# cvlab-kaist/PF3plat

Hardware: AMD Instinct MI355X
Metric: rendered views/sec, 300k Gaussians @ 256x256 (fwd raster); bwd ms and HBM GB/s vs roofline alongside (higher is better)
Workload: dtype f32; 1 GPU; configs[1]: 300000 Gaussians (SH degree 4, 25 coeffs), 1 view 256x256, fwd-only raster, one scene per GPU (seed 2+rank), inputs resident in HBM; launch=eager, parallelism=views sharded 1 scene/GPU x1, camera_setup=excluded (gsr_setup_views runs once before the loop; ~4 us per batch of views), num_pairs_8x8=1252130, max_tile_list=1663

## Files before the change

pf3plat_amd/csrc/gsr_tiles_fwd.h:

```cpp
#pragma once
#include "gsr_common.h"
#include "gsr_binning.h"

namespace gsr {

template <bool kFlip, class KeyPtr>
__device__ __forceinline__ void bitonic_substep(KeyPtr a, int n, int half, int lg, int tid) {
  constexpr int U = 4;
  const int w = 1 << lg;
  for (int tb = tid; tb < half; tb += kSortThreads * U) {
    int ii[U], jj[U];
    unsigned long long x[U], y[U];
    bool act[U];
#pragma unroll
    for (int u = 0; u < U; ++u) {
      const int t = tb + u * kSortThreads;
      const int blk = t >> lg, off = t & (w - 1);
      ii[u] = (blk << (lg + 1)) + off;
      jj[u] = kFlip ? (blk << (lg + 1)) + 2 * w - 1 - off : ii[u] + w;
      act[u] = (t < half) && (jj[u] < n);
      x[u] = act[u] ? a[ii[u]] : 0ull;
      y[u] = act[u] ? a[jj[u]] : 0ull;
    }
#pragma unroll
    for (int u = 0; u < U; ++u)
      if (act[u] && x[u] > y[u]) { a[ii[u]] = y[u]; a[jj[u]] = x[u]; }
  }
}

template <class KeyPtr>
__device__ __forceinline__ void bitonic_block(KeyPtr a, int n, int lgnp, int tid) {
  const int half = 1 << (lgnp - 1);
  for (int lk = 1; lk <= lgnp; ++lk) {
    bitonic_substep<true>(a, n, half, lk - 1, tid);
    __syncthreads();
    for (int lj = lk - 2; lj >= 0; --lj) {
      bitonic_substep<false>(a, n, half, lj, tid);
      __syncthreads();
    }
  }
}

constexpr int kSpanMax = 48;

__device__ __forceinline__ bool block_any(const bool pred, uint32_t* slot) {
  const bool w = __any((int)pred) != 0;
  if ((threadIdx.x & 63) == 0) slot[threadIdx.x >> 6] = w ? 1u : 0u;
  __syncthreads();
  return (slot[0] | slot[1] | slot[2] | slot[3]) != 0u;
}

__device__ __forceinline__ uint32_t block_exclusive_scan(uint32_t v, uint32_t* wave_tot , int tid, uint32_t& total) {
  const int lane = tid & 63, w = tid >> 6;
  const uint32_t s = wave_inclusive_scan_u32(v);
  if (lane == 63) wave_tot[w] = s;
  __syncthreads();
  uint32_t basew = 0;
  total = 0;
#pragma unroll
  for (int k = 0; k < kSortThreads / 64; ++k) {
    const uint32_t x = wave_tot[k];
    basew += (k < w) ? x : 0u;
    total += x;
  }
  return basew + s - v;
}

template <int kLds>
struct SortLds {
  static constexpr int kBuckets = kLds == 2048 ? 2048 : 1024, kBucketBits = kLds == 2048 ? 11 : 10;
  static constexpr int kWords = kLds + kBuckets / 2;
};

template <bool kGather, int kLds>
__device__ __forceinline__ uint2 sort_tile(const Params& p, const uint32_t bid, const int tg, unsigned long long* smem, uint32_t* red,
                                           uint32_t* sInfo) {
  constexpr int kBk = SortLds<kLds>::kBuckets, kBkBits = SortLds<kLds>::kBucketBits, kBpt = kBk / kSortThreads;
  static_assert(kLds == 4096 || kLds == 2048, "bucket geometry");
  unsigned long long* sk = smem;
  uint32_t* hist = reinterpret_cast<uint32_t*>(smem + kLds);
  uint32_t* cur = hist;
  const int tid = threadIdx.x;
  const bool dbg = GSR_ABL(p.d.flags, GSR_FLAG_DEBUG_TIMING);
  unsigned long long* stamp = dbg_stamps(p, 8192 + bid);
  unsigned long long* stamp2 = dbg_stamps(p, 8192 + p.sort_blocks + bid);
  GSR_STAMP(0);
  int n;
  uint32_t obase = 0;
  unsigned long long* keys;
  uint32_t* out;
  if (kGather) {
    const int T = p.g.T, R = p.rows;
    const int v = tg / T, t = tg - v * T;
    if (bid < 1024u) {
      for (int q = 0; q < (int)((bid >> kDephaseShift) % kDephaseGroups); ++q) __builtin_amdgcn_s_sleep(64);
    }
    const uint2* col = p.pair_mat + (size_t)v * R * (T + 8) + t;
    const size_t cstride = (size_t)T + 8;
    const uint32_t* bb = p.blk_base + (size_t)v * R;
    const bool one_stride = R <= kSortThreads;
    uint2 e0 = make_uint2(0u, 0u);
    uint32_t bb0 = 0, cnt_sum = 0, missing = 0;
    if (one_stride) {
      if (tid < R) { e0 = col[(size_t)tid * cstride]; bb0 = bb[tid]; }
      cnt_sum = e0.y;
      missing = (e0.y != 0u && bb0 == 0xffffffffu) ? 1u : 0u;
    } else {
      for (int r = tid; r < R; r += kSortThreads) {
        const uint32_t c = col[(size_t)r * cstride].y;
        cnt_sum += c;
        missing |= (c != 0u && bb[r] == 0xffffffffu) ? 1u : 0u;
      }
    }
    GSR_STAMP2(0);
    uint32_t total;
    const uint32_t start0 = block_exclusive_scan(cnt_sum, red, tid, total);
    __shared__ uint32_t sAnyMissing[kSortThreads / 64];
    const bool any_missing = block_any(missing, sAnyMissing);
    n = (int)total;
    const bool plain = !any_missing && (uint32_t)n <= p.stride && n <= kLds;
    if (!plain && tid == 64 && (uint32_t)n > p.status->max_list) atomicMax(&p.status->max_list, (uint32_t)n);
    if (plain) {
      if (tid == 0) p.ranges[tg] = make_uint2((uint32_t)tg * p.stride, (uint32_t)tg * p.stride + (uint32_t)n);
    } else if (tid == 0) {
      uint32_t rbase = (uint32_t)tg * p.stride, ok = any_missing ? 0u : 1u, scratch = 0;
      if (ok && (uint32_t)n > p.stride) {
        const uint32_t at = atomicAdd(p.tail_counter, (uint32_t)n);
        if (at <= p.tail_cap && (uint32_t)n <= p.tail_cap - at) rbase = p.tail_off + at;
        else ok = 0;
      }
      if (ok && n > kLds) {
        const uint32_t np = ((uint32_t)n + kPage - 1) / kPage;
        const uint32_t first = take_pages(p.page_counter_tiles, p.call_tag, np), half = p.key_pages / 2;
        if (first <= p.key_pages - half && np <= p.key_pages - half - first) scratch = p.pool_off + (half + first) * (uint32_t)kPage;
        else ok = 0;
      }
      if (!ok) p.status->overflow = 1u;
      p.ranges[tg] = ok ? make_uint2(rbase, rbase + (uint32_t)n) : make_uint2(0u, 0u);
      sInfo[0] = rbase; sInfo[1] = ok; sInfo[2] = scratch;
    }
    if (bid == 0) {
      unsigned long long part = 0;
      for (int k = tid; k < p.d.num_views * R; k += kSortThreads) part += p.blk_total[k];
      for (int o = 32; o > 0; o >>= 1) part += __shfl_down(part, o, 64);
      __shared__ unsigned long long sPart[kSortThreads / 64];
      if ((tid & 63) == 0) sPart[tid >> 6] = part;
      __syncthreads();
      if (tid == 0) p.status->num_pairs = sPart[0] + sPart[1] + sPart[2] + sPart[3];
    }
    uint32_t rbase = (uint32_t)tg * p.stride, scratch = 0;
    if (!plain) {
      __syncthreads();
      if (!sInfo[1]) return make_uint2(0u, 0u);
      rbase = sInfo[0]; scratch = sInfo[2];
    }
    obase = rbase;
    if (n == 0) return make_uint2(obase, obase);
    GSR_STAMP2(1);
    out = p.point_list + rbase;
    keys = p.keys + scratch;
    unsigned long long* dst = n > kLds ? keys : sk;
    auto copy_run = [&](const unsigned long long* src, uint32_t cnt, uint32_t start) {
      for (uint32_t j = 0; j < cnt; j += 6) {
        const ull2 a = *reinterpret_cast<const ull2*>(src + j);
        ull2 b = {0ull, 0ull}, c = {0ull, 0ull};
        if (j + 2 < cnt) b = *reinterpret_cast<const ull2*>(src + j + 2);
        if (j + 4 < cnt) c = *reinterpret_cast<const ull2*>(src + j + 4);
        unsigned long long* d = dst + start + j;
        d[0] = a.x;
        if (j + 1 < cnt) d[1] = a.y;
        if (j + 2 < cnt) d[2] = b.x;
        if (j + 3 < cnt) d[3] = b.y;
        if (j + 4 < cnt) d[4] = c.x;
        if (j + 5 < cnt) d[5] = c.y;
      }
    };
    if (one_stride) {
      if (e0.y) copy_run(p.keys + bb0 + e0.x, e0.y, start0);
      __syncthreads();
      GSR_STAMP2(2);
    } else {
      uint32_t carry = 0;
      for (int r0 = 0; r0 < R; r0 += kSortThreads) {
        const int r = r0 + tid;
        const uint2 e = r < R ? col[(size_t)r * cstride] : make_uint2(0u, 0u);
        uint32_t tot;
        const uint32_t start = carry + block_exclusive_scan(e.y, red, tid, tot);
        carry += tot;
        if (e.y) copy_run(p.keys + bb[r] + e.x, e.y, start);
        __syncthreads();
      }
    }
    if (n == 1) {
      if (tid == 0) out[0] = (uint32_t)dst[0];
      return make_uint2(obase, obase + 1u);
    }
  } else {
    const uint2 rg = p.ranges[bid];
    n = (int)(rg.y - rg.x);
    obase = rg.x;
    if (n == 0) return rg;
    keys = p.keys + rg.x;
    out = p.point_list + rg.x;
    if (n == 1) {
      if (tid == 0) out[0] = (uint32_t)keys[0];
      return rg;
    }
  }
  int lgnp = 1;
  while ((1 << lgnp) < n) ++lgnp;
  if (n > kLds) {
    __syncthreads();
    bitonic_block(keys, n, lgnp, tid);
    for (int k = tid; k < n; k += kSortThreads) out[k] = (uint32_t)keys[k];
    return make_uint2(obase, obase + (uint32_t)n);
  }
  constexpr int Q = kLds / kSortThreads;
  unsigned long long kreg[Q];
  uint32_t lo = 0xffffffffu, hi = 0u;
#pragma unroll
  for (int q = 0; q < Q; ++q) {
    const int k = tid + q * kSortThreads;
    kreg[q] = (k < n) ? (kGather ? sk[k] : keys[k]) : ~0ull;
    if (k < n) {
      const uint32_t d = (uint32_t)(kreg[q] >> 32);
      lo = d < lo ? d : lo;
      hi = d > hi ? d : hi;
    }
  }
  GSR_STAMP(1);
  for (int k = tid; k < kBk; k += kSortThreads) hist[k] = 0;
  hi = wave_max_u32(hi);
  lo = ~wave_max_u32(~lo);
  if ((tid & 63) == 0) { red[tid >> 6] = lo; red[4 + (tid >> 6)] = hi; }
  __syncthreads();
  lo = min(min(red[0], red[1]), min(red[2], red[3]));
  hi = max(max(red[4], red[5]), max(red[6], red[7]));
  const uint32_t range = hi - lo;
  const int shift = range < (uint32_t)kBk ? 0 : (32 - __clz((int)range)) - kBkBits;
#pragma unroll
  for (int q = 0; q < Q; ++q)
    if (tid + q * kSortThreads < n) atomicAdd(&hist[((uint32_t)(kreg[q] >> 32) - lo) >> shift], 1u);
  __syncthreads();
  GSR_STAMP(2);
  uint32_t c[kBpt], span = 0, cmax = 0;
#pragma unroll
  for (int q = 0; q < kBpt; ++q) { c[q] = hist[kBpt * tid + q]; span += c[q]; cmax = max(cmax, c[q]); }
  uint32_t total;
  uint32_t start = block_exclusive_scan(span, red, tid, total);
#pragma unroll
  for (int q = 0; q < kBpt; ++q) { cur[kBpt * tid + q] = start; start += c[q]; }
  __shared__ uint32_t sAnyBig[kSortThreads / 64];
  const bool big = block_any(cmax > (uint32_t)kSpanMax, sAnyBig);
  GSR_STAMP(3);
#pragma unroll
  for (int q = 0; q < Q; ++q)
    if (tid + q * kSortThreads < n) {
      const uint32_t slot = atomicAdd(&cur[((uint32_t)(kreg[q] >> 32) - lo) >> shift], 1u);
      sk[slot] = kreg[q];
    }
  __syncthreads();
  GSR_STAMP(4);
  if (!big) {
    for (int k = tid; k < n; k += kSortThreads) {
      const unsigned long long key = sk[k];
      const uint32_t b = ((uint32_t)(key >> 32) - lo) >> shift;
      const int bs = b ? (int)cur[b - 1] : 0, be = (int)cur[b];
      int rank = bs;
      for (int j = bs; j < be; j += 4) {
        const unsigned long long k0 = sk[j], k1 = sk[min(j + 1, be - 1)], k2 = sk[min(j + 2, be - 1)], k3 = sk[min(j + 3, be - 1)];
        rank += (k0 < key ? 1 : 0) + ((j + 1 < be && k1 < key) ? 1 : 0) + ((j + 2 < be && k2 < key) ? 1 : 0) +
                ((j + 3 < be && k3 < key) ? 1 : 0);
      }
      out[rank] = (uint32_t)key;
    }
    GSR_STAMP(5);
    GSR_STAMP(6);
    return make_uint2(obase, obase + (uint32_t)n);
  }
  bitonic_block(sk, n, lgnp, tid);
  __syncthreads();
  GSR_STAMP(5);
  for (int k = tid; k < n; k += kSortThreads) out[k] = (uint32_t)sk[k];
  GSR_STAMP(6);
  return make_uint2(obase, obase + (uint32_t)n);
}


constexpr float kLog2e = 1.4426950408889634f;
constexpr float kLn2 = 0.6931471805599453f;

__device__ __forceinline__ void to_exp2_domain(float4& q0, float4& q1) {
  q0.z = (-0.5f * kLog2e) * q0.z;
  q0.w = (-kLog2e) * q0.w;
  q1.x = (-0.5f * kLog2e) * q1.x;
}
__device__ __forceinline__ float splat_p2(float a2, float b2, float c2, float dx, float dy) {
  const float t = __builtin_fmaf(b2, dy, a2 * dx);
  return __builtin_fmaf(c2 * dy, dy, t * dx);
}

typedef float f2 __attribute__((ext_vector_type(2)));
constexpr int kFwdWaves = 4;
#ifndef GSR_KFS
#define GSR_KFS 8
#endif
constexpr int kFS = GSR_KFS;
constexpr int kFB = kFS * kFwdWaves;
constexpr int kFwdThreads = 64 * kFwdWaves;

__device__ __forceinline__ void stage_batch(const GeomRec* geom, const float4* rgbc, uint32_t n, uint32_t base, int lane,
                                            uint32_t id, bool want_extra, float4& g, float2& g2, float4& c) {
  g = make_float4(0, 0, 0, 0); g2 = make_float2(0, 0); c = make_float4(0, 0, 0, 0);
  if (base + lane < n) {
    const GeomRec* r = geom + id;
    const float4 q0 = r->q0, q1 = r->q1;
    const float4 col = rgbc[id];
    const float ex = want_extra ? q1.z : 0.f;
    g = q0; g2 = make_float2(q1.x, q1.y); c = make_float4(col.x, col.y, col.z, ex);
  }
}

struct BlendLds {
  float4 sXY[4][kFB / 2], sAB[4][kFB / 2], sCO[4][kFB / 2], sRG[4][kFB / 2], sBE[4][kFB / 2];
  float sP[2][kFwdWaves][64];
};
struct BlendFin {
  float sPart[kFwdWaves][5][64];
  uint32_t sLast[kFwdWaves][64];
};

struct BlendAcc {
  float Tb;
  float Tmin;
  f2 CR, CG, CB, CE;
  uint32_t last, consumed;
};

template <bool kExtra, bool kTight = false>
__device__ __forceinline__ bool blend_range(const GeomRec* geom, const float4* rgbc, const uint32_t* plist, const uint32_t n,
                                            const uint32_t b0, const uint32_t nbat, BlendLds& lds, BlendAcc& s, const float pxf,
                                            const float pyf) {
  auto& sXY = lds.sXY; auto& sAB = lds.sAB; auto& sCO = lds.sCO; auto& sRG = lds.sRG; auto& sBE = lds.sBE;
  auto& sP = lds.sP;
  const int wave = __builtin_amdgcn_readfirstlane((int)(threadIdx.x >> 6));
  const int lane = threadIdx.x & 63;
  float Tb = s.Tb, Tmin = s.Tmin;
  f2 al[kFS / 2];
  uint32_t last = s.last, consumed = s.consumed;
  const int e0 = wave * kFS;

  const f2 px2 = {pxf, pxf}, py2 = {pyf, pyf};
  f2 om[kFS / 2];
  auto eval = [&](uint32_t b) {
    const int gb = b & 3;
    f2 P2 = {1.f, 1.f};
#pragma unroll
    for (int u = 0; u < kFS; u += 2) {
      const float4 xy = sXY[gb][(e0 + u) >> 1], ab = sAB[gb][(e0 + u) >> 1], co = sCO[gb][(e0 + u) >> 1];
      const f2 dx = f2{xy.x, xy.y} - px2, dy = f2{xy.z, xy.w} - py2;
      const f2 a2 = {ab.x, ab.y}, b2 = {ab.z, ab.w}, c2 = {co.x, co.y}, o = {co.z, co.w};
      const f2 t = __builtin_elementwise_fma(b2, dy, a2 * dx);
      const f2 p2 = __builtin_elementwise_fma(c2 * dy, dy, t * dx);
      const f2 ao = o * f2{__builtin_amdgcn_exp2f(p2.x), __builtin_amdgcn_exp2f(p2.y)};
      const float alpha0 = fminf(0.99f, ao.x), alpha1 = fminf(0.99f, ao.y);
      const bool keep0 = !(p2.x > 0.f) && !(alpha0 < 1.0f / 255.0f), keep1 = !(p2.y > 0.f) && !(alpha1 < 1.0f / 255.0f);
      al[u >> 1] = f2{keep0 ? alpha0 : 0.f, keep1 ? alpha1 : 0.f};
      om[u >> 1] = f2{1.f, 1.f} - al[u >> 1];
      P2 *= om[u >> 1];
    }
    sP[b & 1][wave][lane] = P2.x * P2.y;
  };
  f2 CR = s.CR, CG = s.CG, CB = s.CB, CE = s.CE;
  auto accum = [&](uint32_t b, float Tf) {
    const int cb = b & 3;
    const bool alive_in = !(Tf < 0.0001f);
    float T = alive_in ? Tf : 0.f;
    float Tn[kFS];
    f2 w[kFS / 2];
    float Tp = T;
#pragma unroll
    for (int u = 0; u < kFS; u += 2) {
      Tn[u] = Tp * om[u >> 1].x;
      Tn[u + 1] = Tn[u] * om[u >> 1].y;
      Tp = Tn[u + 1];
    }
    const bool alive_out = !(Tp < 0.0001f);
    if (__any(alive_in && !alive_out)) {
      float Tq = T;
#pragma unroll
      for (int u = 0; u < kFS; u += 2) {
        const bool alive0 = !(Tn[u] < 0.0001f), alive1 = !(Tn[u + 1] < 0.0001f);
        w[u >> 1] = al[u >> 1] * f2{alive0 ? Tq : 0.f, alive1 ? Tn[u] : 0.f};
        Tq = Tn[u + 1];
        Tmin = alive0 ? Tn[u] : Tmin;
        Tmin = alive1 ? Tn[u + 1] : Tmin;
        last += (uint32_t)alive0 + (uint32_t)alive1;
      }
    } else {
      float Tq = T;
#pragma unroll
      for (int u = 0; u < kFS; u += 2) {
        w[u >> 1] = al[u >> 1] * f2{Tq, Tn[u]};
        Tq = Tn[u + 1];
      }
      Tmin = alive_out ? Tp : Tmin;
      last += alive_out ? (uint32_t)kFS : 0u;
    }
#pragma unroll
    for (int u = 0; u < kFS; u += 2) {
      const float4 rg = sRG[cb][(e0 + u) >> 1], be = sBE[cb][(e0 + u) >> 1];
      CR = __builtin_elementwise_fma(f2{rg.x, rg.y}, w[u >> 1], CR);
      CG = __builtin_elementwise_fma(f2{rg.z, rg.w}, w[u >> 1], CG);
      CB = __builtin_elementwise_fma(f2{be.x, be.y}, w[u >> 1], CB);
      if (kExtra) CE = __builtin_elementwise_fma(f2{be.z, be.w}, w[u >> 1], CE);
    }
    asm volatile("" : "+v"(CR), "+v"(CG), "+v"(CB), "+v"(Tmin), "+v"(last));
    if (kExtra) asm volatile("" : "+v"(CE));
  };
  auto put_records = [&](int sb, float4 q, float2 q2, const float4& c) {
    q.z = (-0.5f * kLog2e) * q.z; q.w = (-kLog2e) * q.w; q2.x = (-0.5f * kLog2e) * q2.x;
    int ln = lane;
    if (kTight) asm volatile("" : "+v"(ln));
    const int o = (ln >> 1) * 4 + (ln & 1);
    float* xy = reinterpret_cast<float*>(sXY[sb]); float* ab = reinterpret_cast<float*>(sAB[sb]);
    float* co = reinterpret_cast<float*>(sCO[sb]); float* rg2 = reinterpret_cast<float*>(sRG[sb]);
    float* be = reinterpret_cast<float*>(sBE[sb]);
    xy[o] = q.x; xy[o + 2] = q.y; ab[o] = q.z; ab[o + 2] = q.w; co[o] = q2.x; co[o + 2] = q2.y;
    rg2[o] = c.x; rg2[o + 2] = c.y; be[o] = c.z; be[o + 2] = c.w;
  };

  bool done = false;
  if (nbat > b0) {
    float4 sg = make_float4(0, 0, 0, 0), sc = sg;
    float2 sg2 = make_float2(0, 0);
    uint32_t id_next = 0;
    int lp = lane;
    if (kTight) asm volatile("" : "+v"(lp));
    const auto list_id = [&](uint32_t b) { return (b * kFB + lp < n) ? plist[b * kFB + lp] : 0u; };
    if (lp < kFB) {
      const uint32_t w = (uint32_t)(wave - (int)b0) & 3u, bw = b0 + w;
      if (w < 2) {
        const uint32_t id0 = list_id(bw), id4 = list_id(bw + 4);
        id_next = list_id(bw + 8);
        if (bw < nbat) {
          stage_batch(geom, rgbc, n, bw * kFB, lane, id0, kExtra, sg, sg2, sc);
          put_records((int)(bw & 3), sg, sg2, sc);
        }
        stage_batch(geom, rgbc, n, (bw + 4) * kFB, lane, id4, kExtra, sg, sg2, sc);
      } else {
        const uint32_t id2 = list_id(bw);
        id_next = list_id(bw + 4);
        stage_batch(geom, rgbc, n, bw * kFB, lane, id2, kExtra, sg, sg2, sc);
      }
    }
    __syncthreads();
    eval(b0);
    __syncthreads();
    for (uint32_t i = b0; i < nbat; ++i) {
      const float P0 = sP[i & 1][0][lane], P1 = sP[i & 1][1][lane], P2 = sP[i & 1][2][lane], P3 = sP[i & 1][3][lane];
      const uint32_t bs = i + 2;
      const bool duty = (wave == (int)(bs & 3)) && (lane < kFB);
      const float t1 = Tb * P0, t2 = t1 * P1, t3 = t2 * P2, t4 = t3 * P3;
      const bool last_batch = __all(t4 < 0.0001f);
      accum(i, wave == 0 ? Tb : wave == 1 ? t1 : wave == 2 ? t2 : t3);
      if (i + 1 < nbat && !last_batch) eval(i + 1);
      if (duty) {
        if (bs < nbat) put_records((int)(bs & 3), sg, sg2, sc);
        if (bs + 4 < nbat) stage_batch(geom, rgbc, n, (bs + 4) * kFB, lane, id_next, kExtra, sg, sg2, sc);
        id_next = list_id(bs + 8);
      }
      Tb = t4;
      consumed = (i + 1) * kFB;
      __syncthreads();
      if (__all(Tb < 0.0001f)) { done = true; break; }
    }
  }
  s.Tb = Tb; s.Tmin = Tmin; s.CR = CR; s.CG = CG; s.CB = CB; s.CE = CE; s.last = last; s.consumed = consumed;
  return done;
}

template <bool kExtra, bool kAlpha = false>
__device__ __forceinline__ bool blend_poisoned(const Params& p, const int v, const int pxi, const int pyi, const bool inside,
                                               const bool known = false) {
  __shared__ uint32_t sAnyOverflow[kFwdThreads / 64];
  if (!known && !block_any(p.status->overflow != 0u, sAnyOverflow)) return false;
  const Grid& g = p.g;
  if (threadIdx.x < 64 && inside) {
    const size_t HW = (size_t)g.H * g.W, pix = (size_t)pyi * g.W + pxi;
    const float qnan = __uint_as_float(0x7fc00000u);
    float* oc = p.out_color + (size_t)v * 3 * HW;
    oc[pix] = qnan; oc[HW + pix] = qnan; oc[2 * HW + pix] = qnan;
    if (kExtra) p.out_extra[(size_t)v * HW + pix] = qnan;
    if (kAlpha) p.out_alpha[(size_t)v * HW + pix] = qnan;
    p.final_T[(size_t)v * HW + pix] = 1.f;
    p.n_contrib[(size_t)v * HW + pix] = 0u;
  }
  return true;
}

template <bool kExtra, bool kAlpha = false>
__device__ __forceinline__ void blend_finish(const Params& p, const int v, const int t, const uint32_t n, BlendFin& lds, const BlendAcc& s,
                                             const int pxi, const int pyi, const bool inside, const float bg0, const float bg1,
                                             const float bg2) {
  auto& sPart = lds.sPart; auto& sLast = lds.sLast;
  const Grid& g = p.g;
  const int wave = threadIdx.x >> 6, lane = threadIdx.x & 63;
  float C0 = s.CR.x + s.CR.y, C1 = s.CG.x + s.CG.y, C2 = s.CB.x + s.CB.y, E = s.CE.x + s.CE.y;
  sPart[wave][0][lane] = C0; sPart[wave][1][lane] = C1; sPart[wave][2][lane] = C2;
  if (kExtra) sPart[wave][3][lane] = E;
  sPart[wave][4][lane] = s.Tmin;
  sLast[wave][lane] = s.last;
  __syncthreads();
  if (wave == 0) {
    if (lane == 0) p.tile_total[(size_t)v * g.T + t] = min(s.consumed, n);
    if (inside) {
      float T = s.Tmin;
      uint32_t last = s.last;
#pragma unroll
      for (int h = 1; h < kFwdWaves; ++h) {
        C0 += sPart[h][0][lane]; C1 += sPart[h][1][lane]; C2 += sPart[h][2][lane];
        if (kExtra) E += sPart[h][3][lane];
        T = fminf(T, sPart[h][4][lane]);
        last += sLast[h][lane];
      }
      const size_t HW = (size_t)g.H * g.W, pix = (size_t)pyi * g.W + pxi;
      p.final_T[(size_t)v * HW + pix] = T;
      if (kAlpha) p.out_alpha[(size_t)v * HW + pix] = 1.f - T;
      p.n_contrib[(size_t)v * HW + pix] = min(last, n);
      float* oc = p.out_color + (size_t)v * 3 * HW;
      oc[pix] = C0 + T * bg0;
      oc[HW + pix] = C1 + T * bg1;
      oc[2 * HW + pix] = C2 + T * bg2;
      if (kExtra) p.out_extra[(size_t)v * HW + pix] = E;
    }
  }
}

template <bool kExtra, bool kAlpha = false>
__device__ __forceinline__ void blend_tile(const Params& p, const int v, const int t, const uint2 rg, BlendLds& lds) {
  const Grid& g = p.g;
  const int lane = threadIdx.x & 63;
  const int tx = t % g.sgx, ty = t / g.sgx;
  const int pxi = tx * 8 + (lane & 7), pyi = ty * 8 + (lane >> 3);
  const bool inside = pxi < g.W && pyi < g.H;
  const uint32_t n = rg.y - rg.x;
  typedef const __attribute__((address_space(4))) float* cfptr;
  cfptr camc = reinterpret_cast<cfptr>(reinterpret_cast<uintptr_t>(p.views + __builtin_amdgcn_readfirstlane(v)));
  const float bg0 = camc[37], bg1 = camc[38], bg2 = camc[39];
  if (blend_poisoned<kExtra, kAlpha>(p, v, pxi, pyi, inside)) return;
  const bool dbg = GSR_ABL(p.d.flags, GSR_FLAG_DEBUG_TIMING);
  unsigned long long tm0 = 0, rt0 = 0;
  if (dbg) { tm0 = __builtin_readcyclecounter(); rt0 = __builtin_amdgcn_s_memrealtime(); }
  BlendAcc acc;
  acc.Tb = inside ? 1.f : 0.f; acc.Tmin = 1.f;
  acc.CR = f2{0.f, 0.f}; acc.CG = acc.CR; acc.CB = acc.CR; acc.CE = acc.CR;
  acc.last = 0; acc.consumed = 0;
  (void)blend_range<kExtra>(p.geom + (size_t)v * p.d.num_gaussians, p.rgbc + (size_t)v * p.d.num_gaussians, p.point_list + rg.x, n, 0u,
                            (n + kFB - 1) / kFB, lds, acc, (float)pxi, (float)pyi);
  if (dbg && threadIdx.x == 0) {
    unsigned long long* o = dbg_stamps(p, 24576 + (size_t)v * g.T + t);
    const unsigned hw = (__builtin_amdgcn_s_getreg(4 | (0 << 6) | (15 << 11)) & 0xffffu) |
                        ((__builtin_amdgcn_s_getreg(20 | (0 << 6) | (15 << 11)) & 0xfu) << 16);
    o[0] = tm0; o[1] = ((unsigned long long)hw << 32); o[2] = __builtin_readcyclecounter();
    o[3] = (rt0 << 32) | (__builtin_amdgcn_s_memrealtime() & 0xffffffffull);
  }
  blend_finish<kExtra, kAlpha>(p, v, t, n, *reinterpret_cast<BlendFin*>(&lds + 1), acc, pxi, pyi, inside, bg0, bg1, bg2);
}

#ifndef GSR_TF_WAVES
#define GSR_TF_WAVES 6
#endif
#ifndef GSR_WINDOWED_SHORT
#define GSR_WINDOWED_SHORT 600
#endif
template <bool kGather, int kLds, bool kExtra, bool kAlpha = false>
__global__ __launch_bounds__(kFwdThreads, (kLds == 2048 && kGather && !kExtra) ? GSR_TF_WAVES : 4) void k_tile_fwd(const Params p) {
  static_assert(kSortThreads == kFwdThreads, "one workgroup shape for the two phases");
  constexpr int kSortWords = SortLds<kLds>::kWords, kBlendWords = (int)((sizeof(BlendLds) + sizeof(BlendFin) + 7) / 8);
  __shared__ __attribute__((aligned(16))) unsigned long long smem[kSortWords > kBlendWords ? kSortWords : kBlendWords];
  __shared__ uint32_t red[8];
  __shared__ uint32_t sInfo[4];
  const uint32_t bid = blockIdx.x;
  const int tg = kGather ? fwd_tile_of(p, fwd_tile_word(p, bid)) : (int)bid;
  __builtin_amdgcn_s_setprio(2);
  const uint2 rg = sort_tile<kGather, kLds>(p, bid, tg, smem, red, sInfo);
  __builtin_amdgcn_s_setprio(0);
  if (bid == 0 && threadIdx.x == 0) *p.page_counter = (unsigned long long)p.call_tag << 32;
  __syncthreads();
  const int v = tg / p.g.T;
  blend_tile<kExtra, kAlpha>(p, v, tg - v * p.g.T, rg, *reinterpret_cast<BlendLds*>(smem));
  if (kGather && threadIdx.x == 64 && rg.y - rg.x > p.status->max_list) atomicMax(&p.status->max_list, rg.y - rg.x);
}

#ifndef GSR_PREFIX
#define GSR_PREFIX 512
#endif
#ifndef GSR_DEPHASE_SLEEP
#define GSR_DEPHASE_SLEEP 16
#endif
#ifndef GSR_LONG_RUN
#define GSR_LONG_RUN 24
#endif
constexpr int kPrefix = GSR_PREFIX;
static_assert(kPrefix % kFB == 0 && kPrefix >= 2 * kFB, "the prefix is whole batches");

__device__ __forceinline__ uint2 sort_tile_general_2048(const Params& p, const uint32_t bid, const int tg, unsigned long long* smem, uint32_t* red, uint32_t* sInfo) {
  return sort_tile<true, 2048>(p, bid, tg, smem, red, sInfo);
}
__device__ __forceinline__ void bitonic_whole_list(unsigned long long* sk, uint32_t* out, const int n) {
  int lgnp = 1;
  while ((1 << lgnp) < n) ++lgnp;
  bitonic_block(sk, n, lgnp, (int)threadIdx.x);
  for (int k = threadIdx.x; k < n; k += kSortThreads) out[k] = (uint32_t)sk[k];
}

#ifndef GSR_PF_COMPACT_MIN_TILES
#define GSR_PF_COMPACT_MIN_TILES (5 * kCUs)
#endif
template <bool kExtra, bool kCompact, bool kAlpha = false>
__global__ __launch_bounds__(kFwdThreads, kCompact ? 6 : 4) void k_tile_fwd_prefix(const Params p) {
  constexpr int kLds = 2048;
  constexpr int kBk = kCompact ? 1024 : SortLds<kLds>::kBuckets, kBkBits = kCompact ? 10 : SortLds<kLds>::kBucketBits, kBpt = kBk / kSortThreads;
  constexpr int Q = kLds / kSortThreads;
  constexpr int kCounterWords = kCompact ? kBk / 4 : kBk / 2;
  constexpr int kBlendWordsP = (int)((sizeof(BlendLds) + 7) / 8);
  constexpr int kFastWords = kLds + kCounterWords + (kCompact ? kBlendWordsP : 0);
  __shared__ __attribute__((aligned(16))) unsigned long long smem[kFastWords > SortLds<kLds>::kWords ? kFastWords : SortLds<kLds>::kWords];
  __shared__ __attribute__((aligned(16))) unsigned long long blds_own[kCompact ? 2 : kBlendWordsP];
  BlendLds& blds = *reinterpret_cast<BlendLds*>(kCompact ? smem + kLds + kCounterWords : blds_own);
  __shared__ uint32_t red[8];
  __shared__ uint32_t sInfo[4];
  __shared__ uint32_t sCount, sLongRuns, sLongKeys;
  const uint32_t bid = blockIdx.x;
  const int tid = threadIdx.x, lane = tid & 63, wave = tid >> 6;
  const uint32_t tile_word = kCompact ? (uint32_t)xcd_remap((int)bid, (int)p.sort_blocks) : fwd_tile_word(p, bid);
  uint32_t overflow_early = 0;
  if (tid == 0) overflow_early = p.status->overflow;
  unsigned long long* sk = smem;
  uint32_t* hist = reinterpret_cast<uint32_t*>(smem + kLds);
  uint32_t* cur = hist;
  auto bump = [&](uint32_t b) -> uint32_t {
    if (!kCompact) return atomicAdd(&cur[b], 1u);
    const uint32_t sh = (b & 1u) * 16u;
    return (atomicAdd(&cur[b >> 1], 1u << sh) >> sh) & 0xffffu;
  };
  auto cur_of = [&](uint32_t b) -> uint32_t { return kCompact ? (cur[b >> 1] >> ((b & 1u) * 16u)) & 0xffffu : cur[b]; };
  const bool dbg = GSR_ABL(p.d.flags, GSR_FLAG_DEBUG_TIMING);
  unsigned long long* stamp = dbg_stamps(p, 8192 + bid);
  unsigned long long* stamp2 = dbg_stamps(p, 8192 + p.sort_blocks + bid);
  __builtin_amdgcn_s_setprio(2);
  GSR_STAMP(0);
  const int T = p.g.T, R = p.rows;
  if (bid < 1024u)
    for (int q = 0; q < (int)((bid >> kDephaseShift) % kDephaseGroups); ++q) __builtin_amdgcn_s_sleep(GSR_DEPHASE_SLEEP);
  const int tg = fwd_tile_of(p, tile_word);
  const int v = tg / T, t = tg - v * T;
  uint2 e0 = make_uint2(0u, 0u);
  uint32_t bb0 = 0;
  if (tid < R) {
    e0 = p.pair_mat[((size_t)v * R + tid) * ((size_t)T + 8) + t];
    bb0 = p.blk_base[(size_t)v * R + tid];
  }
  for (int k = tid; k < (kCompact ? kBk / 2 : kBk); k += kSortThreads) hist[k] = 0;
  if (tid == 0) { sCount = 0; sLongRuns = 0; sLongKeys = 0; }
  __syncthreads();
  GSR_STAMP2(0);
  const bool has = e0.y != 0u, miss = has && bb0 == 0xffffffffu;
  const uint32_t incl = wave_inclusive_scan_u32(e0.y);
  uint32_t wbase = 0;
  if (lane == 63 && incl) wbase = atomicAdd(&sCount, incl);
  wbase = (uint32_t)__builtin_amdgcn_readlane((int)wbase, 63);
  const uint32_t start0 = wbase + incl - e0.y;
  const bool fits = start0 + e0.y <= (uint32_t)kLds;
  GSR_STAMP2(1);
  uint32_t lo = 0xffffffffu, hi = 0u;
  auto take = [&](unsigned long long* d, unsigned long long key) {
    *d = key;
    const uint32_t dep = (uint32_t)(key >> 32);
    lo = dep < lo ? dep : lo;
    hi = dep > hi ? dep : hi;
  };
  constexpr uint32_t kLongRun = GSR_LONG_RUN;
  uint4* ldesc = reinterpret_cast<uint4*>(&blds);
  static_assert(sizeof(BlendLds) >= (size_t)(kLds / GSR_LONG_RUN + 1) * 16, "descriptors of the long runs fit the blend's area");
  const bool is_long = has && !miss && fits && e0.y > kLongRun;
  if (__any((int)is_long)) {
    const uint32_t lcnt = is_long ? e0.y : 0u;
    const uint32_t lincl = wave_inclusive_scan_u32(lcnt);
    const unsigned long long lmask = __ballot((int)is_long);
    uint32_t kbase = 0, dbase = 0;
    if (lane == 63) {
      kbase = atomicAdd(&sLongKeys, lincl);
      dbase = atomicAdd(&sLongRuns, (uint32_t)__popcll(lmask));
    }
    kbase = (uint32_t)__builtin_amdgcn_readlane((int)kbase, 63);
    dbase = (uint32_t)__builtin_amdgcn_readlane((int)dbase, 63);
    if (is_long)
      ldesc[dbase + (uint32_t)__popcll(lmask & ((1ull << lane) - 1ull))] = make_uint4(bb0 + e0.x, start0, e0.y, kbase + lincl - lcnt);
  }
  if (has && !miss && fits && !is_long) {
    const unsigned long long* src = p.keys + bb0 + e0.x;
    unsigned long long* d0 = sk + start0;
    for (uint32_t j = 0; j < e0.y; j += 6) {
      const ull2 a = *reinterpret_cast<const ull2*>(src + j);
      ull2 b = {0ull, 0ull}, c = {0ull, 0ull};
      if (j + 2 < e0.y) b = *reinterpret_cast<const ull2*>(src + j + 2);
      if (j + 4 < e0.y) c = *reinterpret_cast<const ull2*>(src + j + 4);
      unsigned long long* d = d0 + j;
      take(d, a.x);
      if (j + 1 < e0.y) take(d + 1, a.y);
      if (j + 2 < e0.y) take(d + 2, b.x);
      if (j + 3 < e0.y) take(d + 3, b.y);
      if (j + 4 < e0.y) take(d + 4, c.x);
      if (j + 5 < e0.y) take(d + 5, c.y);
    }
  }
  hi = wave_max_u32(hi);
  lo = ~wave_max_u32(~lo);
  if (lane == 0) { red[wave] = lo; red[4 + wave] = hi; }
  if (tid == 0) sInfo[3] = overflow_early;
  __shared__ uint32_t sAnyBad[kSortThreads / 64];
  const bool bad = block_any(miss || (has && !fits), sAnyBad);
  if (sLongRuns != 0u) {
    const uint32_t nruns = sLongRuns, nkeys = sLongKeys;
    constexpr int QL = kLds / kSortThreads;
    unsigned long long kv[QL];
    uint32_t dst[QL];
    uint32_t r = 0;
    uint4 dsc = ldesc[0];
#pragma unroll
    for (int q = 0; q < QL; ++q) {
      const uint32_t f = (uint32_t)tid + (uint32_t)q * kSortThreads;
      dst[q] = 0xffffffffu;
      kv[q] = 0ull;
      if (f < nkeys) {
        if (!(f >= dsc.w && f - dsc.w < dsc.z)) {
          for (r = 0; r < nruns; ++r) {
            dsc = ldesc[r];
            if (f >= dsc.w && f - dsc.w < dsc.z) break;
          }
        }
        kv[q] = p.keys[(size_t)dsc.x + (f - dsc.w)];
        dst[q] = dsc.y + (f - dsc.w);
      }
    }
    uint32_t lo2 = 0xffffffffu, hi2 = 0u;
#pragma unroll
    for (int q = 0; q < QL; ++q)
      if (dst[q] != 0xffffffffu) {
        sk[dst[q]] = kv[q];
        const uint32_t dep = (uint32_t)(kv[q] >> 32);
        lo2 = dep < lo2 ? dep : lo2;
        hi2 = dep > hi2 ? dep : hi2;
      }
    hi2 = wave_max_u32(hi2);
    lo2 = ~wave_max_u32(~lo2);
    if (lane == 0) { red[wave] = min(red[wave], lo2); red[4 + wave] = max(red[4 + wave], hi2); }
    __syncthreads();
  }
  GSR_STAMP2(2);
  GSR_STAMP(1);
  uint32_t n = sCount, ranked = 0, obase = (uint32_t)tg * p.stride;
  uint32_t dlo = 0;
  int shift = 0;
  bool fast_path = false;
  bool bucketed = false;
  if (bad || n > p.stride) {
    __syncthreads();
    const uint2 rg = sort_tile_general_2048(p, bid, tg, smem, red, sInfo);
    obase = rg.x; n = rg.y - rg.x; ranked = n;
  } else {
    if (tid == 0) p.ranges[tg] = make_uint2(obase, obase + n);
    fast_path = true;
    uint32_t* out = p.point_list + obase;
    if (n == 1) {
      if (tid == 0) out[0] = (uint32_t)sk[0];
      ranked = 1;
    } else if (n > 1) {
      dlo = min(min(red[0], red[1]), min(red[2], red[3]));
      const uint32_t dhi = max(max(red[4], red[5]), max(red[6], red[7]));
      const uint32_t range = dhi - dlo;
      shift = range < (uint32_t)kBk ? 0 : (32 - __clz((int)range)) - kBkBits;
      unsigned long long kreg[Q];
#pragma unroll
      for (int q = 0; q < Q; ++q) {
        const int k = tid + q * kSortThreads;
        kreg[q] = (k < (int)n) ? sk[k] : ~0ull;
        if (k < (int)n) (void)bump(((uint32_t)(kreg[q] >> 32) - dlo) >> shift);
      }
      __syncthreads();
      GSR_STAMP(2);
      uint32_t c[kBpt], span = 0, cmax = 0;
#pragma unroll
      for (int q = 0; q < kBpt; ++q) { c[q] = cur_of((uint32_t)(kBpt * tid + q)); span += c[q]; cmax = max(cmax, c[q]); }
      uint32_t total;
      uint32_t start = block_exclusive_scan(span, red, tid, total);
      if (kCompact) {
#pragma unroll
        for (int q = 0; q < kBpt; q += 2) {
          const uint32_t s0 = start, s1 = start + c[q];
          cur[(kBpt * tid + q) >> 1] = s0 | (s1 << 16);
          start = s1 + c[q + 1];
        }
      } else {
#pragma unroll
        for (int q = 0; q < kBpt; ++q) { cur[kBpt * tid + q] = start; start += c[q]; }
      }
      __shared__ uint32_t sAnyBig2[kSortThreads / 64];
      const bool big = block_any(cmax > (uint32_t)kSpanMax, sAnyBig2);
      GSR_STAMP(3);
      if (big) {
        bitonic_whole_list(sk, out, (int)n);
        ranked = n;
      } else {
#pragma unroll
        for (int q = 0; q < Q; ++q)
          if (tid + q * kSortThreads < (int)n) {
            const uint32_t slot = bump(((uint32_t)(kreg[q] >> 32) - dlo) >> shift);
            sk[slot] = kreg[q];
          }
        __syncthreads();
        GSR_STAMP(4);
        ranked = n;
        if (!(p.d.flags & GSR_FLAG_FULL_LISTS) && n > (uint32_t)(kPrefix + kPrefix / 4))
          ranked = cur_of(((uint32_t)(sk[kPrefix - 1] >> 32) - dlo) >> shift);
        bucketed = true;
      }
    }
  }
  auto rank_positions = [&](uint32_t k0, uint32_t k1) {
    uint32_t* out = p.point_list + obase;
    for (int k = (int)k0 + tid; k < (int)k1; k += kSortThreads) {
      const unsigned long long key = sk[k];
      const uint32_t b = ((uint32_t)(key >> 32) - dlo) >> shift;
      const int bs = b ? (int)cur_of(b - 1) : 0, be = (int)cur_of(b);
      int rank = bs;
      for (int j = bs; j < be; j += 4) {
        const unsigned long long k0_ = sk[j], k1_ = sk[min(j + 1, be - 1)], k2_ = sk[min(j + 2, be - 1)], k3_ = sk[min(j + 3, be - 1)];
        rank += (k0_ < key ? 1 : 0) + ((j + 1 < be && k1_ < key) ? 1 : 0) + ((j + 2 < be && k2_ < key) ? 1 : 0) +
                ((j + 3 < be && k3_ < key) ? 1 : 0);
      }
      out[rank] = (uint32_t)key;
    }
  };
  if (bucketed) rank_positions(0u, ranked);
  GSR_STAMP(5);
  GSR_STAMP(6);
  __builtin_amdgcn_s_setprio(0);
  if (bid == 0 && tid == 0) *p.page_counter = (unsigned long long)p.call_tag << 32;
  __syncthreads();
  const Grid& g = p.g;
  const int tx = t % g.sgx, ty = t / g.sgx;
  const int pxi = tx * 8 + (lane & 7), pyi = ty * 8 + (lane >> 3);
  const bool inside = pxi < g.W && pyi < g.H;
  typedef const __attribute__((address_space(4))) float* cfptr;
  cfptr camc = reinterpret_cast<cfptr>(reinterpret_cast<uintptr_t>(p.views + __builtin_amdgcn_readfirstlane(v)));
  const float bg0 = camc[37], bg1 = camc[38], bg2 = camc[39];
  auto report_length = [&]() {
    if (fast_path && tid == 64 && n > p.status->max_list) atomicMax(&p.status->max_list, n);
    if (fast_path && bid == 0) {
      unsigned long long part = 0;
      for (int k = tid; k < p.d.num_views * R; k += kSortThreads) part += p.blk_total[k];
      for (int o = 32; o > 0; o >>= 1) part += __shfl_down(part, o, 64);
      __shared__ unsigned long long sPartSum[kSortThreads / 64];
      if (lane == 0) sPartSum[wave] = part;
      __syncthreads();
      if (tid == 0) p.status->num_pairs = sPartSum[0] + sPartSum[1] + sPartSum[2] + sPartSum[3];
    }
  };
  if (fast_path ? (sInfo[3] != 0u && blend_poisoned<kExtra, kAlpha>(p, v, pxi, pyi, inside, true))
                                          : blend_poisoned<kExtra, kAlpha>(p, v, pxi, pyi, inside)) {
    report_length();
    return;
  }
  unsigned long long tm0 = 0, rt0 = 0;
  if (dbg) { tm0 = __builtin_readcyclecounter(); rt0 = __builtin_amdgcn_s_memrealtime(); }
  BlendAcc acc;
  acc.Tb = inside ? 1.f : 0.f; acc.Tmin = 1.f;
  acc.CR = f2{0.f, 0.f}; acc.CG = acc.CR; acc.CB = acc.CR; acc.CE = acc.CR;
  acc.last = 0; acc.consumed = 0;
  const GeomRec* geom = p.geom + (size_t)v * p.d.num_gaussians;
  const float4* rgbc = p.rgbc + (size_t)v * p.d.num_gaussians;
  const uint32_t* plist = p.point_list + obase;
  const uint32_t nbat = (n + kFB - 1) / kFB;
  uint32_t b0 = 0;
#pragma clang loop unroll(disable)
  for (int pass = 0; pass < 2; ++pass) {
    const bool whole = ranked >= n;
    const uint32_t b1 = whole ? nbat : ranked / kFB;
    bool done = blend_range<kExtra, kCompact>(geom, rgbc, plist, whole ? n : b1 * kFB, b0, b1, blds, acc, (float)pxi, (float)pyi);
    done = done || whole || __all(acc.Tb < 0.0001f);
    if (done) break;
    __builtin_amdgcn_s_setprio(2);
    rank_positions(ranked, n);
    __builtin_amdgcn_s_setprio(0);
    ranked = n;
    b0 = b1;
    __syncthreads();
  }
  if (dbg && tid == 0) {
    unsigned long long* o = dbg_stamps(p, 24576 + (size_t)v * g.T + t);
    const unsigned hw = (__builtin_amdgcn_s_getreg(4 | (0 << 6) | (15 << 11)) & 0xffffu) |
                        ((__builtin_amdgcn_s_getreg(20 | (0 << 6) | (15 << 11)) & 0xfu) << 16);
    o[0] = tm0; o[1] = ((unsigned long long)hw << 32); o[2] = __builtin_readcyclecounter();
    o[3] = (rt0 << 32) | (__builtin_amdgcn_s_memrealtime() & 0xffffffffull);
  }
  if (kCompact) {
    int ln = lane;
    asm volatile("" : "+v"(ln));
    const int qx = tx * 8 + (ln & 7), qy = ty * 8 + (ln >> 3);
    blend_finish<kExtra, kAlpha>(p, v, t, n, *reinterpret_cast<BlendFin*>(smem), acc, qx, qy, qx < g.W && qy < g.H, bg0, bg1, bg2);
  } else {
    blend_finish<kExtra, kAlpha>(p, v, t, n, *reinterpret_cast<BlendFin*>(smem), acc, pxi, pyi, inside, bg0, bg1, bg2);
  }
  report_length();
  (void)sInfo;
}

}
```

Before: 19460 views/s.

## Prime first blend batches from ranking step and widen key-run copy

During rank_positions in the non-compact fused sort+blend path, threads that place one of the first two batches' ids stage that Gaussian's geometry and color records directly into the blend LDS. They also hand the first ten batches of ids over through the shared sP area. The primed blend_range then skips the global point_list reads and the staging of batches 0 and 1. Separately, the non-compact key-run copy now issues a configurable number of 16-byte loads per iteration (default 18 keys) instead of 6. The changes aim to cut the latency between sort and blend, at the cost of extra register pressure and LDS aliasing of sP that must stay consistent with the blend's own use.

```diff
diff --git a/pf3plat_amd/csrc/gsr_tiles_fwd.h b/pf3plat_amd/csrc/gsr_tiles_fwd.h
--- a/pf3plat_amd/csrc/gsr_tiles_fwd.h
+++ b/pf3plat_amd/csrc/gsr_tiles_fwd.h
@@ -325,6 +325,17 @@
   float4 sXY[4][kFB / 2], sAB[4][kFB / 2], sCO[4][kFB / 2], sRG[4][kFB / 2], sBE[4][kFB / 2];
   float sP[2][kFwdWaves][64];
 };
+__device__ __forceinline__ void park_record(BlendLds& lds, const int sb, const int e, float4 q, float2 q2, const float4& c) {
+  q.z = (-0.5f * kLog2e) * q.z; q.w = (-kLog2e) * q.w; q2.x = (-0.5f * kLog2e) * q2.x;
+  const int o = (e >> 1) * 4 + (e & 1);
+  float* xy = reinterpret_cast<float*>(lds.sXY[sb]); float* ab = reinterpret_cast<float*>(lds.sAB[sb]);
+  float* co = reinterpret_cast<float*>(lds.sCO[sb]); float* rg2 = reinterpret_cast<float*>(lds.sRG[sb]);
+  float* be = reinterpret_cast<float*>(lds.sBE[sb]);
+  xy[o] = q.x; xy[o + 2] = q.y; ab[o] = q.z; ab[o + 2] = q.w; co[o] = q2.x; co[o + 2] = q2.y;
+  rg2[o] = c.x; rg2[o + 2] = c.y; be[o] = c.z; be[o + 2] = c.w;
+}
+constexpr int kPrimedIds = 10 * kFB;
+static_assert(sizeof(uint32_t) * kPrimedIds <= sizeof(BlendLds::sP), "the handed-over ids fit the segment products' area");
 struct BlendFin {
   float sPart[kFwdWaves][5][64];
   uint32_t sLast[kFwdWaves][64];
@@ -337,7 +348,7 @@
   uint32_t last, consumed;
 };
 
-template <bool kExtra, bool kTight = false>
+template <bool kExtra, bool kTight = false, bool kPrimed = false>
 __device__ __forceinline__ bool blend_range(const GeomRec* geom, const float4* rgbc, const uint32_t* plist, const uint32_t n,
                                             const uint32_t b0, const uint32_t nbat, BlendLds& lds, BlendAcc& s, const float pxf,
                                             const float pyf) {
@@ -438,7 +449,16 @@
     int lp = lane;
     if (kTight) asm volatile("" : "+v"(lp));
     const auto list_id = [&](uint32_t b) { return (b * kFB + lp < n) ? plist[b * kFB + lp] : 0u; };
-    if (lp < kFB) {
+    if constexpr (kPrimed) {
+      if (lp < kFB) {
+        const uint32_t* sid = reinterpret_cast<const uint32_t*>(&sP[0][0][0]);
+        const auto handed_id = [&](uint32_t b) { return (b * kFB + lp < n) ? sid[b * kFB + lp] : 0u; };
+        const uint32_t w = (uint32_t)(wave - (int)b0) & 3u, bq = b0 + (w < 2 ? w + 4 : w);
+        const uint32_t idq = handed_id(bq);
+        id_next = handed_id(bq + 4);
+        stage_batch(geom, rgbc, n, bq * kFB, lane, idq, kExtra, sg, sg2, sc);
+      }
+    } else if (lp < kFB) {
       const uint32_t w = (uint32_t)(wave - (int)b0) & 3u, bw = b0 + w;
       if (w < 2) {
         const uint32_t id0 = list_id(bw), id4 = list_id(bw + 4);
@@ -601,6 +621,9 @@
 #endif
 #ifndef GSR_LONG_RUN
 #define GSR_LONG_RUN 24
+#endif
+#ifndef GSR_RUN_STEP
+#define GSR_RUN_STEP 18
 #endif
 constexpr int kPrefix = GSR_PREFIX;
 static_assert(kPrefix % kFB == 0 && kPrefix >= 2 * kFB, "the prefix is whole batches");
@@ -699,7 +722,27 @@
     if (is_long)
       ldesc[dbase + (uint32_t)__popcll(lmask & ((1ull << lane) - 1ull))] = make_uint4(bb0 + e0.x, start0, e0.y, kbase + lincl - lcnt);
   }
-  if (has && !miss && fits && !is_long) {
+  if (!kCompact && has && !miss && fits && !is_long) {
+    constexpr uint32_t kRunStep = GSR_RUN_STEP;
+    static_assert(kRunStep % 2 == 0 && kRunStep >= 6, "whole 16-byte loads");
+    const unsigned long long* src = p.keys + bb0 + e0.x;
+    unsigned long long* d0 = sk + start0;
+    for (uint32_t j = 0; j < e0.y; j += kRunStep) {
+      ull2 r[kRunStep / 2];
+#pragma unroll
+      for (uint32_t u = 0; u < kRunStep / 2; ++u) {
+        r[u] = ull2{0ull, 0ull};
+        if (j + 2 * u < e0.y) r[u] = *reinterpret_cast<const ull2*>(src + j + 2 * u);
+      }
+      unsigned long long* d = d0 + j;
+#pragma unroll
+      for (uint32_t u = 0; u < kRunStep / 2; ++u) {
+        if (j + 2 * u < e0.y) take(d + 2 * u, r[u].x);
+        if (j + 2 * u + 1 < e0.y) take(d + 2 * u + 1, r[u].y);
+      }
+    }
+  }
+  if (kCompact && has && !miss && fits && !is_long) {
     const unsigned long long* src = p.keys + bb0 + e0.x;
     unsigned long long* d0 = sk + start0;
     for (uint32_t j = 0; j < e0.y; j += 6) {
@@ -829,8 +872,15 @@
       }
     }
   }
-  auto rank_positions = [&](uint32_t k0, uint32_t k1) {
+  static_assert(kSpanMax + 2 * kFB <= kSortThreads, "a thread holds at most one record of batches 0 and 1");
+  auto rank_positions = [&](uint32_t k0, uint32_t k1, const bool prime) {
+    const GeomRec* geom = p.geom + (size_t)v * p.d.num_gaussians;
+    const float4* rgbc = p.rgbc + (size_t)v * p.d.num_gaussians;
     uint32_t* out = p.point_list + obase;
+    uint32_t* sid = reinterpret_cast<uint32_t*>(&blds.sP[0][0][0]);
+    float4 hg = make_float4(0, 0, 0, 0), hc = hg;
+    float2 hg2 = make_float2(0, 0);
+    int held = -1;
     for (int k = (int)k0 + tid; k < (int)k1; k += kSortThreads) {
       const unsigned long long key = sk[k];
       const uint32_t b = ((uint32_t)(key >> 32) - dlo) >> shift;
@@ -842,9 +892,21 @@
                 ((j + 3 < be && k3_ < key) ? 1 : 0);
       }
       out[rank] = (uint32_t)key;
+      if (prime) {
+        if (rank < kPrimedIds) sid[rank] = (uint32_t)key;
+        if (rank < 2 * kFB) {
+          stage_batch(geom, rgbc, 1u, 0u, 0, (uint32_t)key, kExtra, hg, hg2, hc);
+          held = rank;
+        }
+      }
+    }
+    if (prime) {
+      if (held >= 0) park_record(blds, held / kFB, held % kFB, hg, hg2, hc);
+      if (tid < 2 * kFB && tid >= (int)k1) park_record(blds, tid / kFB, tid % kFB, make_float4(0, 0, 0, 0), make_float2(0, 0), make_float4(0, 0, 0, 0));
     }
   };
-  if (bucketed) rank_positions(0u, ranked);
+  const bool primed = !kCompact && bucketed;
+  if (bucketed) rank_positions(0u, ranked, primed);
   GSR_STAMP(5);
   GSR_STAMP(6);
   __builtin_amdgcn_s_setprio(0);
@@ -889,11 +951,13 @@
   for (int pass = 0; pass < 2; ++pass) {
     const bool whole = ranked >= n;
     const uint32_t b1 = whole ? nbat : ranked / kFB;
-    bool done = blend_range<kExtra, kCompact>(geom, rgbc, plist, whole ? n : b1 * kFB, b0, b1, blds, acc, (float)pxi, (float)pyi);
+    const uint32_t nb = whole ? n : b1 * kFB;
+    bool done = (primed && pass == 0) ? blend_range<kExtra, kCompact, !kCompact>(geom, rgbc, plist, nb, b0, b1, blds, acc, (float)pxi, (float)pyi)
+                                      : blend_range<kExtra, kCompact>(geom, rgbc, plist, nb, b0, b1, blds, acc, (float)pxi, (float)pyi);
     done = done || whole || __all(acc.Tb < 0.0001f);
     if (done) break;
     __builtin_amdgcn_s_setprio(2);
-    rank_positions(ranked, n);
+    rank_positions(ranked, n, false);
     __builtin_amdgcn_s_setprio(0);
     ranked = n;
     b0 = b1;
```

After: 19910 views/s, median of 6. 1.02x the previous value.
